# Giuseppe5/brevitas

Measured on AMD Instinct MI355X. Metric: Gelem/s fused int8 fake-quant fwd+bwd, per-channel, [256,512,56,56], higher is better.
Workload: dtype bf16

## Files before the change

brevitas_amd/_native.py:

```python
import ctypes
import os

import torch

_PKG = os.path.dirname(os.path.abspath(__file__))
LIB_PATH = os.environ.get('BREVITAS_AMD_LIB') or os.path.join(_PKG, 'libbvq.so')

F32, BF16, F16 = 0, 1, 2
ROUND, FLOOR, CEIL, ROUND_TO_ZERO, DPU_ROUND = range(5)
(OP_ROUND, OP_FLOOR, OP_CEIL, OP_ROUND_TO_ZERO, OP_DPU_ROUND, OP_BINARY_SIGN, OP_TERNARY_SIGN,
 OP_ABS) = range(8)
STAT_ABSMAX, STAT_MINMAX = 0, 1
SCALAR_OPMATH, SCALAR_CAST = 0, 1
OUT_DEQUANT, OUT_INT = 0, 1
MATCH_ABS, MATCH_VALUE = 0, 1
MATCH_FIRST = 16
PRE_NONE, PRE_RELU, PRE_SIGMOID, PRE_TANH = 0, 1, 2, 3
CODES_I32, CODES_I8, CODES_U8 = 0, 1, 2
CLUSTER_FORCE_FALLBACK = 1
_CODES_TORCH = {CODES_I32: torch.int32, CODES_I8: torch.int8, CODES_U8: torch.uint8}
ABI_VERSION = 2

_DTYPES = {torch.float32: F32, torch.bfloat16: BF16, torch.float16: F16}

EXPORTS = (
    'bvq_abi_version', 'bvq_last_error', 'bvq_unary', 'bvq_stats_pre', 'bvq_scalar_clamp', 'bvq_tensor_clamp',
    'bvq_tensor_clamp_bwd', 'bvq_abs_binary_sign_grad_bwd', 'bvq_stats_workspace_bytes', 'bvq_stats',
    'bvq_absmax_scale', 'bvq_running_stats_update', 'bvq_scale_from_stat', 'bvq_shard_pack', 'bvq_shard_unpack', 'bvq_abs_moments_workspace_bytes', 'bvq_abs_moments',
    'bvq_abs_affine_bwd', 'bvq_kth_workspace_bytes', 'bvq_kth_value', 'bvq_kth_pair', 'bvq_kth_passes',
    'bvq_kth_hist_offset', 'bvq_kth_begin', 'bvq_kth_hist', 'bvq_kth_pick', 'bvq_kth_finish', 'bvq_stat_bwd', 'bvq_tie_info_bytes', 'bvq_stat_tie_scan', 'bvq_stat_tie_apply', 'bvq_stat_tie_apply_dscale', 'bvq_fakequant_fwd', 'bvq_stats_fakequant_fwd_workspace_bytes', 'bvq_stats_fakequant_fwd',
    'bvq_fakequant_bwd_workspace_bytes', 'bvq_fakequant_bwd_stats_workspace_bytes', 'bvq_fakequant_bwd_stats', 'bvq_fakequant_bwd',
    'bvq_learned_scale', 'bvq_fakequant_bwd_learned', 'bvq_variant_fwd', 'bvq_variant_bwd_workspace_bytes', 'bvq_variant_bwd',
    'bvq_fakequant_fwd_bounds', 'bvq_fakequant_bwd_bounds', 'bvq_histc', 'bvq_absmax_scale_running', 'bvq_selftest_div_f16r',
    'bvq_kthw_plan', 'bvq_kthw_begin', 'bvq_kthw_hist', 'bvq_kthw_pick', 'bvq_kthw_finish',
    'bvq_absmax_onepass_supported', 'bvq_absmax_scale_onepass', 'bvq_fakequant_bwd_stats_onepass_supported',
    'bvq_fakequant_bwd_stats_onepass', 'bvq_scale_from_stat_running', 'bvq_fakequant_bwd_shard',
    'bvq_shard_unpack_deposit', 'bvq_absmax_list_supported', 'bvq_absmax_scale_list', 'bvq_weight_list_supported',
    'bvq_weight_quant_list_fwd', 'bvq_weight_quant_list_bwd_workspace_bytes', 'bvq_weight_quant_list_bwd',
    'bvq_absmax_fakequant_cluster_supported', 'bvq_absmax_fakequant_cluster', 'bvq_selftest_pre_op')


class QuantDesc(ctypes.Structure):
    _fields_ = [
        ('outer', ctypes.c_int64), ('channels', ctypes.c_int64), ('inner', ctypes.c_int64),
        ('x_dtype', ctypes.c_int32), ('ct_dtype', ctypes.c_int32), ('scale_dtype', ctypes.c_int32),
        ('zp_dtype', ctypes.c_int32), ('scale_per_channel', ctypes.c_int32),
        ('zp_per_channel', ctypes.c_int32), ('qmin', ctypes.c_float), ('qmax', ctypes.c_float),
        ('round_mode', ctypes.c_int32), ('scalar_mode', ctypes.c_int32), ('clamp_ste', ctypes.c_int32),
        ('out_kind', ctypes.c_int32), ('pre_op', ctypes.c_int32), ('codes_dtype', ctypes.c_int32)]


class VariantDesc(ctypes.Structure):
    _fields_ = [
        ('outer', ctypes.c_int64), ('channels', ctypes.c_int64), ('inner', ctypes.c_int64), ('kind', ctypes.c_int32),
        ('x_dtype', ctypes.c_int32), ('ct_dtype', ctypes.c_int32), ('scale_dtype', ctypes.c_int32),
        ('zp_dtype', ctypes.c_int32), ('scale_per_channel', ctypes.c_int32), ('round_mode', ctypes.c_int32),
        ('clamp_ste', ctypes.c_int32), ('scalar_mode', ctypes.c_int32), ('qmin', ctypes.c_float),
        ('qmax', ctypes.c_float), ('threshold', ctypes.c_float), ('trunc_scale', ctypes.c_float)]


VAR_BINARY, VAR_CLAMPED_BINARY, VAR_TERNARY, VAR_DECOUPLED, VAR_TRUNC = range(5)

WEIGHT_LIST_MAX = 16


class WeightItem(ctypes.Structure):
    _fields_ = [
        ('x', ctypes.c_void_p), ('y', ctypes.c_void_p), ('stat', ctypes.c_void_p), ('scale', ctypes.c_void_p),
        ('g', ctypes.c_void_p), ('dx', ctypes.c_void_p), ('dscale', ctypes.c_void_p), ('channels', ctypes.c_int64),
        ('inner', ctypes.c_int64), ('min_val', ctypes.c_double), ('int_threshold', ctypes.c_double),
        ('qmin', ctypes.c_float), ('qmax', ctypes.c_float), ('use_min', ctypes.c_int32), ('clamp_ste', ctypes.c_int32)]

# ... 51 lines not shown
        'bvq_kth_pair': (i32, [i32, i32, vp, i64, i64, i64, i64, i64, vp, vp, i64, vp]),
        'bvq_kth_passes': (i32, [i32]),
        'bvq_kth_hist_offset': (i64, [i32, i64, i32]),
        'bvq_kth_begin': (i32, [i32, i64, i32, i64, dbl, vp, i64, vp]),
        'bvq_kth_hist': (i32, [i32, i32, vp, i64, i64, i64, i32, vp, i64, vp]),
        'bvq_kth_pick': (i32, [i32, i64, i32, i32, dbl, vp, i64, vp]),
        'bvq_kth_finish': (i32, [i32, i32, i64, vp, vp, i64, vp]),
        'bvq_kthw_plan': (i32, [i32, i32, i32, vp, vp]),
        'bvq_kthw_begin': (i32, [i32, i32, vp, i64, vp]),
        'bvq_kthw_hist': (i32, [i32, i32, vp, i64, i32, vp, i64, vp]),
        'bvq_kthw_pick': (i32, [i32, i32, i32, i32, i64, dbl, vp, i64, vp]),
        'bvq_kthw_finish': (i32, [i32, i32, vp, vp, i64, vp]),
        'bvq_tie_info_bytes': (i64, [i64]),
        'bvq_stat_tie_scan': (i32, [i32, i32, vp, vp, i64, i64, i64, vp, vp, vp]),
        'bvq_stat_tie_apply': (i32, [i32, i32, i32, vp, vp, vp, vp, vp, vp, i64, i64, i64, i32, vp]),
        'bvq_stat_tie_apply_dscale': (i32, [i32, i32, vp, vp, vp, i32, dbl, i32, vp, vp, vp, i64, i64, i64, vp]),
        'bvq_fakequant_bwd': (i32, [ctypes.POINTER(QuantDesc), vp, vp, vp, vp, vp, vp, vp, vp, vp, vp, i64, vp]),
        'bvq_learned_scale': (i32, [i32, vp, i64, dbl, i32, dbl, i32, vp, vp]),
        'bvq_histc': (i32, [i32, vp, i64, vp, i32, vp, vp]),
        'bvq_selftest_div_f16r': (i32, [vp, i32, vp, i32, vp, vp]),
        'bvq_selftest_pre_op': (i32, [i32, i32, vp, vp, vp, vp, i64, vp]),
        'bvq_fakequant_fwd_bounds': (i32, [ctypes.POINTER(QuantDesc), vp, vp, vp, vp, vp, vp]),
        'bvq_fakequant_bwd_bounds': (i32, [ctypes.POINTER(QuantDesc), vp, vp, vp, vp, vp, vp, vp, vp, vp, i64, vp]),
        'bvq_variant_fwd': (i32, [ctypes.POINTER(VariantDesc), vp, vp, vp, vp, vp, vp, vp]),
        'bvq_variant_bwd_workspace_bytes': (i64, [ctypes.POINTER(VariantDesc)]),
        'bvq_variant_bwd': (i32, [ctypes.POINTER(VariantDesc), vp, vp, vp, vp, vp, vp, vp, vp, vp, vp, i64, vp]),
        'bvq_weight_list_supported': (i32, [i32, i32, i32, vp, i64]),
        'bvq_weight_quant_list_fwd': (i32, [i32, i32, i32, i32, vp, vp]),
        'bvq_weight_quant_list_bwd_workspace_bytes': (i64, [i32, i32, vp]),
        'bvq_weight_quant_list_bwd': (i32, [i32, i32, i32, i32, i32, vp, vp, i64, vp, i64, vp]),
        'bvq_absmax_fakequant_cluster_supported': (i64, [ctypes.POINTER(QuantDesc), vp, vp]),
        'bvq_absmax_fakequant_cluster': (i32, [ctypes.POINTER(QuantDesc), vp, dbl, i32, dbl, vp, vp, i32, vp, dbl, i32, vp,
                                               vp, i64, i32, vp, vp]),
        'bvq_fakequant_bwd_learned': (i32, [ctypes.POINTER(QuantDesc), vp, vp, vp, vp, vp, vp, vp, i32, dbl, i32, dbl, vp, vp, vp, i64, vp]),
    }
    for name, (res, args) in sig.items():
        fn = getattr(lib, name, None)
        if fn is None:
            if strict:
                raise ImportError('brevitas_amd: %s does not export %s' % (path, name))
            continue
        fn.restype = res
        fn.argtypes = args
    ver = lib.bvq_abi_version()
    if ver != ABI_VERSION:
        raise ImportError('brevitas_amd: libbvq.so has ABI %d, this package needs %d' % (ver, ABI_VERSION))
    return lib


lib = _load()


def last_error():
    return lib.bvq_last_error().decode()


def check(rc, what):
    if rc != 0:
        raise BvqError('%s failed (%d): %s' % (what, rc, last_error()))


def dtype_code(dtype):
    try:
        return _DTYPES[dtype]
    except KeyError:
        raise BvqError('brevitas_amd: unsupported dtype %s (float32, bfloat16, float16)' % dtype)
# ... 197 lines not shown
            _timer.before('bvq_fakequant_fwd')
        check(lib.bvq_fakequant_fwd(ctypes.byref(desc), ptr(x), ptr(scale), ptr(zp), ptr(y), ptr(codes),
                                    stream_ptr(dev)), 'bvq_fakequant_fwd')
        if _timer is not None:
            _timer.after('bvq_fakequant_fwd')
    if not want_y:
        return codes
    return (y, codes) if want_codes else y


def stats_fakequant_fwd(desc, x, min_val, int_threshold, scale_dtype):
    dev = require_device(x)
    assert x.is_contiguous()
    y = torch.empty_like(x)
    wsb = int(lib.bvq_stats_fakequant_fwd_workspace_bytes(ctypes.byref(desc), ptr(x), ptr(y)))
    if wsb <= 0:
        return None
    channels = int(desc.channels) if (desc.scale_per_channel and desc.channels > 1) else 1
    stat = torch.empty(channels, dtype=x.dtype, device=dev)
    scale = torch.empty(channels, dtype=scale_dtype, device=dev)
    ws = torch.empty(wsb, dtype=torch.uint8, device=dev)
    with _DeviceGuard(dev):
        if _timer is not None:
            _timer.before('bvq_stats_fakequant_fwd')
        check(lib.bvq_stats_fakequant_fwd(ctypes.byref(desc), ptr(x), float(min_val or 0.0), int(bool(min_val)),
                                          float(int_threshold), ptr(stat), ptr(scale), ptr(y), ptr(ws), wsb,
                                          stream_ptr(dev)), 'bvq_stats_fakequant_fwd')
        if _timer is not None:
            _timer.after('bvq_stats_fakequant_fwd')
    return stat, scale, y


def absmax_fakequant_cluster(desc, x, min_val, int_threshold, scale_dtype, running=None, momentum=0.0,
                             first_batch=False, flags=0, fallbacks=None):
    dev = require_device(x)
    assert x.is_contiguous()
    y = torch.empty_like(x)
    words = int(lib.bvq_absmax_fakequant_cluster_supported(ctypes.byref(desc), ptr(x), ptr(y)))
    if words <= 0:
        return None
    with _DeviceGuard(dev):
        st = stream_ptr(dev)
        arrive = arrival_buffer(dev, st, words)
        if arrive is None:
            return None
        stat = torch.empty(desc.channels, dtype=x.dtype, device=dev)
        scale = torch.empty(desc.channels, dtype=scale_dtype, device=dev)
        if _timer is not None:
            _timer.before('bvq_stats_fakequant_fwd')
        check(lib.bvq_absmax_fakequant_cluster(
            ctypes.byref(desc), ptr(x), float(min_val or 0.0), int(bool(min_val)), float(int_threshold), ptr(stat),
            ptr(scale), dtype_code(running.dtype) if running is not None else 0, ptr(running), float(momentum),
            int(first_batch), ptr(y), ptr(arrive), arrive.numel(), int(flags), ptr(fallbacks), st),
            'bvq_absmax_fakequant_cluster')
        if _timer is not None:
            _timer.after('bvq_stats_fakequant_fwd')
    return stat, scale, y


def absmax_scale_list(xs, outers, channels, inners, min_val, int_threshold, scale_dtype):
    dev = require_device(*xs)
    n = len(xs)
    dt = dtype_code(xs[0].dtype)
    for x, o, i in zip(xs, outers, inners):
        assert x.is_contiguous() and x.dtype == xs[0].dtype and x.numel() == o * channels * i
    ptrs = (ctypes.c_void_p * n)(*[x.data_ptr() for x in xs])
    oa = (ctypes.c_int64 * n)(*outers)
    ia = (ctypes.c_int64 * n)(*inners)
    if not lib.bvq_absmax_list_supported(dt, n, ptrs, oa, channels, ia):
        return None
    with _DeviceGuard(dev):
        st = stream_ptr(dev)
        arrive = ws = None
        if channels > 1:
            arrive = arrival_buffer(dev, st, max(2 * channels, 18))
            if arrive is None:
                return None
        else:
            ws = torch.empty(1 << 14, dtype=torch.uint8, device=dev)
        stat = torch.empty(channels, dtype=xs[0].dtype, device=dev)
        scale = torch.empty(channels, dtype=scale_dtype, device=dev)
        check(lib.bvq_absmax_scale_list(dt, n, ptrs, oa, channels, ia, ptr(stat), float(min_val or 0.0),
                                        int(bool(min_val)), float(int_threshold), dtype_code(scale_dtype), ptr(scale),
                                        ptr(arrive), arrive.numel() if arrive is not None else 0, ptr(ws),
                                        ws.numel() if ws is not None else 0, st), 'bvq_absmax_scale_list')
    return stat, scale

# ... 578 lines not shown
```

brevitas_amd/csrc/bvq_fakequant_fwd.hip:

```cpp

#include "bvq_act.h"
#include "bvq_fakequant.h"
#include "bvq_stat_epilogue.h"

namespace bvq {

template <typename CT, int RM, bool ZP0, typename Div>
__device__ __forceinline__ float fwd_elem(float xf, const Div& div, float s, float z, float qmin,
                                          float qmax, bool out_int, int mode, float& q_out) {
  float t = rnd<CT>(div(xf));
  t = ZP0 ? t + 0.f : rnd<CT>(t + z);
  t = do_round<CT, RM>(t, mode);
  const float q = clamp_where(t, qmin, qmax);
  q_out = q;
  if (out_int) return q;
  return ZP0 ? rnd<CT>(q * s) : rnd<CT>(rnd<CT>(q - z) * s);
}

template <typename CT, int RM, bool ZP0, typename Div, typename S>
__device__ __forceinline__ f2 fwd_elem2(f2 xf, const Div& div, S s, S z, float qmin, float qmax,
                                        bool out_int, int mode, f2& q_out) {
  f2 t = rnd2<CT>(div(xf));
  t = ZP0 ? t + 0.f : rnd2<CT>(t + z);
  t = do_round2<CT, RM>(t, mode);
// ... 243 lines not shown
  int32_t use_min, scale_dtype, scale_pc, scalar_cast, round_mode, pre_relu;
};

template <typename T>
__device__ __forceinline__ float scale_from_key(uint32_t key, bool use_min, float min_val, float int_threshold,
                                                int scale_dtype, float& stat) {
  if constexpr (elem<T>::id == BVQ_F16)
    stat = (float)__builtin_bit_cast(f16_t, (uint16_t)key);
  else
    stat = __builtin_bit_cast(float, key);
  const float thr = (use_min && stat < min_val) ? min_val : stat;
  float s = thr / int_threshold;
  if (scale_dtype == BVQ_BF16)
    s = rnd<bf16_t>(s);
  else if (scale_dtype == BVQ_F16)
    s = rnd<f16_t>(s);
  return s;
}
template <typename T>
__device__ __forceinline__ void store_stat_scale(void* stat_out, void* scale_out, int scale_dtype, int32_t c,
                                                 float stat, float s) {
  if constexpr (elem<T>::id == BVQ_F32)
    reinterpret_cast<float*>(stat_out)[c] = stat;
  else
    reinterpret_cast<T*>(stat_out)[c] = (T)stat;
  if (scale_dtype == BVQ_F32)
    reinterpret_cast<float*>(scale_out)[c] = s;
  else if (scale_dtype == BVQ_BF16)
    reinterpret_cast<bf16_t*>(scale_out)[c] = (bf16_t)s;
  else
    reinterpret_cast<f16_t*>(scale_out)[c] = (f16_t)s;
}

template <typename T, int RM, bool PRE, typename Div>
__device__ __forceinline__ void fused_quantize(const vec_t<T, elem<T>::vec> (&xv)[kFusedSlots], const bool (&ok)[kFusedSlots],
                                               T* __restrict__ yp, int lane, const Div& div, float s,
                                               float qmin, float qmax, int mode) {
  constexpr int VEC = elem<T>::vec;
  constexpr bool ZP0 = sizeof(T) == 2;
#pragma unroll
  for (int j = 0; j < kFusedSlots; ++j) {
    if (ok[j]) {
      vec_t<T, VEC> yv;
#pragma unroll
      for (int k = 0; k < VEC; k += 2) {
        f2 xf = widen2<T>(xv[j].v[k], xv[j].v[k + 1]);
        if constexpr (PRE) xf = relu2(xf);
        f2 q2;
        const f2 r = fwd_elem2<T, RM, ZP0>(xf, div, s, 0.f, qmin, qmax, false, mode, q2);
        pack2<T>(r, yv.v[k], yv.v[k + 1]);
      }
      store_vec<T, VEC, true>(yp + (int64_t)(lane + kWave * j) * VEC, yv);
    }
  }
}

__global__ void fused_zero_kernel(uint32_t* p, int64_t n) {
  const int64_t i = (int64_t)blockIdx.x * blockDim.x + threadIdx.x;
  if (i < n) p[i] = 0u;
}

__device__ __forceinline__ void fused_slice(const FusedArgs& a, int q, int lane, int& r, int& sl, bool (&ok)[kFusedSlots]) {
  const bool active = q < a.slices;
  r = active ? q / a.spr : 0;
  sl = active ? q - r * a.spr : 0;
  const int nch = active ? (a.cpr - sl * kFusedSliceChunks < kFusedSliceChunks ? a.cpr - sl * kFusedSliceChunks
                                                                              : kFusedSliceChunks)
                         : 0;
#pragma unroll
  for (int j = 0; j < kFusedSlots; ++j) ok[j] = lane + kWave * j < nch;
}

template <typename T>
__device__ __forceinline__ void fused_load(const FusedArgs& a, int32_t c, int r, int sl, const bool (&ok)[kFusedSlots],
                                           int lane, vec_t<T, elem<T>::vec> (&xv)[kFusedSlots]) {
  constexpr int VEC = elem<T>::vec;
  const int64_t base = ((int64_t)r * a.channels + c) * a.inner + (int64_t)sl * kFusedSliceChunks * VEC;
  const T* __restrict__ xp = reinterpret_cast<const T*>(a.x) + base;
#pragma unroll
  for (int j = 0; j < kFusedSlots; ++j)
    xv[j] = load_vec<T, VEC, true>(ok[j] ? xp + (int64_t)(lane + kWave * j) * VEC : reinterpret_cast<const T*>(a.x));
}

template <typename T>
__device__ __forceinline__ uint32_t fused_key(const FusedArgs& a, const vec_t<T, elem<T>::vec> (&xv)[kFusedSlots],
                                              const bool (&ok)[kFusedSlots]) {
  uint32_t m = 0;
#pragma unroll
  for (int j = 0; j < kFusedSlots; ++j) {
    if (ok[j]) {
#pragma unroll
      for (int k = 0; k < elem<T>::vec; ++k) {
        const uint32_t b = a.pre_relu ? pre_abs_bits<T, true>(xv[j].v[k]) : pre_abs_bits<T, false>(xv[j].v[k]);
        m = b > m ? b : m;
      }
    }
  }
  return m;
}

template <typename T, int RM>
__device__ __forceinline__ void fused_apply(const FusedArgs& a, int32_t c, int r, int sl,
                                            const vec_t<T, elem<T>::vec> (&xv)[kFusedSlots], const bool (&ok)[kFusedSlots],
                                            float s, float qmin, float qmax, int lane) {
  constexpr int VEC = elem<T>::vec;
  const int64_t base = ((int64_t)r * a.channels + c) * a.inner + (int64_t)sl * kFusedSliceChunks * VEC;
  T* __restrict__ yp = reinterpret_cast<T*>(a.y) + base;
  const int mode = a.round_mode;
  if constexpr (elem<T>::id == BVQ_BF16) {
    if (bf16_scale_ok(s)) {
      const DivBf16 div{1.0f / s};
      if (a.pre_relu)
        fused_quantize<T, RM, true>(xv, ok, yp, lane, div, s, qmin, qmax, mode);
      else
        fused_quantize<T, RM, false>(xv, ok, yp, lane, div, s, qmin, qmax, mode);
      return;
    }
  }
  if constexpr (elem<T>::id == BVQ_F16) {
    if (f16_scale_ok(s)) {
      const DivF16R div{s, 1.0f / s};
      if (a.pre_relu)
        fused_quantize<T, RM, true>(xv, ok, yp, lane, div, s, qmin, qmax, mode);
      else
        fused_quantize<T, RM, false>(xv, ok, yp, lane, div, s, qmin, qmax, mode);
      return;
    }
  }
  const DivExact div{s};
  if (a.pre_relu)
    fused_quantize<T, RM, true>(xv, ok, yp, lane, div, s, qmin, qmax, mode);
  else
    fused_quantize<T, RM, false>(xv, ok, yp, lane, div, s, qmin, qmax, mode);
}

template <typename T, int RM>
// ... 33 lines not shown
    fused_channel<T, RM>(a, c, r, sl, ok, qmin, qmax, wave, lane, nwaves, sh_max, sh_stat);
}

struct FusedListArgs {
  FusedArgs a[BVQ_WEIGHT_LIST_MAX];
  int32_t start[BVQ_WEIGHT_LIST_MAX + 1];
  int32_t n;
};
static_assert(sizeof(FusedListArgs) <= 4096, "kernel arguments are limited to 4 KiB");

template <typename T, int RM>
__global__ __launch_bounds__(kFusedMaxWaves * kWave) void fused_list_fakequant_kernel(FusedListArgs la) {
  __shared__ uint32_t sh_max[kFusedMaxWaves];
  __shared__ uint32_t sh_stat;
  const int lane = threadIdx.x & 63;
  const int wave = __builtin_amdgcn_readfirstlane((int)(threadIdx.x >> 6));
  const int nwaves = (int)(blockDim.x >> 6);
  int p = -1, r = 0, sl = 0;
  bool ok[kFusedSlots];
  float qmin = 0.f, qmax = 0.f;
  for (int32_t pair = blockIdx.x; pair < la.start[la.n]; pair += gridDim.x) {
    if (p < 0 || pair >= la.start[p + 1]) {
      if (p < 0) p = 0;
      while (p + 1 < la.n && pair >= la.start[p + 1]) ++p;
      fused_slice(la.a[p], wave, lane, r, sl, ok);
      qmin = rnd<T>(la.a[p].qmin);
      qmax = rnd<T>(la.a[p].qmax);
    }
    fused_channel<T, RM>(la.a[p], pair - la.start[p], r, sl, ok, qmin, qmax, wave, lane, nwaves, sh_max, sh_stat);
  }
}


#ifndef BVQ_CLUSTER_WAVES
#define BVQ_CLUSTER_WAVES 16
#endif
#ifndef BVQ_CLUSTER_WAVES_PER_CU
#define BVQ_CLUSTER_WAVES_PER_CU 16
#endif
#ifndef BVQ_CLUSTER_PREFETCH
#define BVQ_CLUSTER_PREFETCH 1
#endif
constexpr int kClusterWaves = BVQ_CLUSTER_WAVES;
constexpr int kClusterWavesPerCu = BVQ_CLUSTER_WAVES_PER_CU;
constexpr bool kClusterPrefetch = BVQ_CLUSTER_PREFETCH != 0;
constexpr int kClusterMaxMembers = kWave;
constexpr uint32_t kClusterTag = 0x80000000u;
constexpr uint64_t kClusterBudgetTicks = 200000;
static_assert(kClusterWaves >= 1 && kClusterWaves * kWave <= 1024, "BVQ_CLUSTER_WAVES");

struct ClusterArgs {
  FusedArgs f;
  ScaleEpilogue ep;
  void* stat_out;
  int32_t in_dtype;
  uint32_t* key;
  uint32_t* dep;
  uint32_t* fallbacks;
  int32_t members, nclusters, force_fallback;
};

template <typename T, int RM>
__global__ __launch_bounds__(kClusterWaves * kWave, kClusterWavesPerCu / 4) void cluster_absmax_fakequant_kernel(ClusterArgs ca) {
  constexpr int VEC = elem<T>::vec;
  __shared__ uint32_t sh_max[kClusterWaves];
  __shared__ uint32_t sh_stat, sh_ok;
  const FusedArgs& a = ca.f;
  const int lane = threadIdx.x & 63;
  const int wave = __builtin_amdgcn_readfirstlane((int)(threadIdx.x >> 6));
  const int32_t members = ca.members;
  const int32_t member = (int32_t)blockIdx.x % members, cluster = (int32_t)blockIdx.x / members;
  int r, sl;
  bool ok[kFusedSlots];
  fused_slice(a, member * kClusterWaves + wave, lane, r, sl, ok);
  const float qmin = rnd<T>(a.qmin), qmax = rnd<T>(a.qmax);
  int32_t c = cluster;
  if (c >= a.channels) return;
  vec_t<T, VEC> xv[kFusedSlots];
  fused_load<T>(a, c, r, sl, ok, lane, xv);
  for (; c < a.channels; c += ca.nclusters) {
    const uint32_t m = wave_max_u32(fused_key<T>(a, xv, ok));
    if (lane == 0) sh_max[wave] = m;
    __syncthreads();
    uint32_t* const keys = ca.key + (int64_t)c * members;
    if (wave == 0) {
      uint32_t bm = 0;
      for (int w = 0; w < kClusterWaves; ++w) bm = sh_max[w] > bm ? sh_max[w] : bm;
      if (lane == 0) __hip_atomic_store(keys + member, bm | kClusterTag, __ATOMIC_RELAXED, __HIP_MEMORY_SCOPE_AGENT);
    }
    const int32_t cn = c + ca.nclusters;
    vec_t<T, VEC> xn[kFusedSlots];
    if (kClusterPrefetch && cn < a.channels) fused_load<T>(a, cn, r, sl, ok, lane, xn);
    if (wave == 0) {
      bool done = false;
      uint32_t v = 0;
      if (!ca.force_fallback) {
        const uint64_t t0 = __builtin_amdgcn_s_memrealtime();
        for (;;) {
          v = lane < members ? __hip_atomic_load(keys + lane, __ATOMIC_RELAXED, __HIP_MEMORY_SCOPE_AGENT) : kClusterTag;
          if (__all((v & kClusterTag) != 0)) {
            done = true;
            break;
          }
          if (__builtin_amdgcn_s_memrealtime() - t0 > kClusterBudgetTicks) break;
          __builtin_amdgcn_s_sleep(2);
        }
      }
      v = wave_max_u32(v) & ~kClusterTag;
      if (lane == 0) {
        sh_stat = v;
        sh_ok = done ? 1u : 0u;
      }
    }
    __syncthreads();
    if (!sh_ok) {
      uint32_t fm = 0;
      for (int q = wave; q < a.slices; q += kClusterWaves) {
        int fr, fsl;
        bool fok[kFusedSlots];
        fused_slice(a, q, lane, fr, fsl, fok);
        const T* xp = reinterpret_cast<const T*>(a.x) + ((int64_t)fr * a.channels + c) * a.inner +
                      (int64_t)fsl * kFusedSliceChunks * VEC;
        for (int j = 0; j < kFusedSlots; ++j) {
          if (!fok[j]) break;
          const vec_t<T, VEC> u = load_vec<T, VEC, false>(xp + (int64_t)(lane + kWave * j) * VEC);
#pragma unroll
          for (int k = 0; k < VEC; ++k) {
            const uint32_t b = a.pre_relu ? pre_abs_bits<T, true>(u.v[k]) : pre_abs_bits<T, false>(u.v[k]);
            fm = b > fm ? b : fm;
          }
        }
      }
      fm = wave_max_u32(fm);
      if (lane == 0) sh_max[wave] = fm;
      __syncthreads();
      if (threadIdx.x == 0) {
        uint32_t bm = 0;
        for (int w = 0; w < kClusterWaves; ++w) bm = sh_max[w] > bm ? sh_max[w] : bm;
        sh_stat = bm;
        if (ca.fallbacks) __hip_atomic_fetch_add(ca.fallbacks, 1u, __ATOMIC_RELAXED, __HIP_MEMORY_SCOPE_AGENT);
      }
      __syncthreads();
    }
    const uint32_t key = sh_stat;
    uint32_t before = 0;
    if (wave == 0) {
      if (lane == 0) {
        if (!sh_ok) asm volatile("s_waitcnt vmcnt(0)" ::: "memory");
        before = __hip_atomic_fetch_add(ca.dep + c, 1u, __ATOMIC_RELAXED, __HIP_MEMORY_SCOPE_AGENT);
      }
    }
    float stat;
    const float s = scale_from_key<T>(key, a.use_min, a.min_val, a.int_threshold, a.scale_dtype, stat);
    if (member == 0 && threadIdx.x == 0) absmax_epilogue(ca.stat_out, ca.in_dtype, ca.in_dtype, ca.ep, c, key);
    fused_apply<T, RM>(a, c, r, sl, xv, ok, s, qmin, qmax, lane);
    if (wave == 0) {
      before = __builtin_amdgcn_readfirstlane(before);
      if (before + 1 == (uint32_t)members) {
        if (lane < members) __hip_atomic_store(keys + lane, 0u, __ATOMIC_RELAXED, __HIP_MEMORY_SCOPE_AGENT);
        if (lane == 0) __hip_atomic_store(ca.dep + c, 0u, __ATOMIC_RELAXED, __HIP_MEMORY_SCOPE_AGENT);
      }
    }
    if (cn < a.channels) {
      if constexpr (kClusterPrefetch) {
#pragma unroll
        for (int j = 0; j < kFusedSlots; ++j) xv[j] = xn[j];
      } else {
        fused_load<T>(a, cn, r, sl, ok, lane, xv);
      }
    }
  }
}

}

using namespace bvq;

static int fakequant_fwd_impl(const bvq_quant_desc* d, const void* x, const void* scale, const void* zp, void* y,
                             void* codes, const float* bounds, bvq_stream_t stream) {
  int rc = validate(d, true);
  if (rc) return rc;
  const bool act = d->pre_op >= BVQ_PRE_SIGMOID;
  if (act && (codes || bounds || !y || d->out_kind != BVQ_OUT_DEQUANT || d->x_dtype != d->ct_dtype)) {
    set_error("bvq_fakequant_fwd: pre_op %d needs the dequantized output in x's dtype, no codes, no device bounds",
              d->pre_op);
    return BVQ_ERR_UNSUPPORTED;
  }
  const int64_t n = d->outer * d->channels * d->inner;
  if (n == 0) return BVQ_OK;
  if (!x || !scale || !zp || (!y && !codes)) {
    set_error("bvq_fakequant_fwd: null pointer");
    return BVQ_ERR_INVALID;
  }
  if (y && !codes && !bounds && !act) {
    const ColsPlan cp = cols_quant_plan(d, x, y, nullptr, true, false, kColsFwdVec16);
    if (cp.ok) {
      ColsQuantArgs ca = {};
      fill_cols_args(ca, cp, d);
      ca.x = x;
      ca.y = y;
      ca.scale = scale;
      ca.zp = zp;
      hipStream_t cst = (hipStream_t)stream;
      const bool cnt = n * (int64_t)(2 * dtype_size(d->x_dtype)) >= nt_threshold_bytes();
      rc = with_cols_variant(d, cnt, [&](auto t, auto rm, auto ntc) {
// ... 146 lines not shown
  a.pre_relu = d->pre_op == BVQ_PRE_RELU;
  return a;
}

extern "C" int bvq_stats_fakequant_fwd(const bvq_quant_desc* d, const void* x, double min_val, int use_min,
                                       double int_threshold, void* stat_out, void* scale_out, void* y,
                                       void* workspace, int64_t workspace_bytes, bvq_stream_t stream) {
  int rc = validate(d);
  if (rc) return rc;
  if (!x || !y || !stat_out || !scale_out || !workspace) {
    set_error("bvq_stats_fakequant_fwd: null pointer");
    return BVQ_ERR_INVALID;
  }
  hipStream_t st = (hipStream_t)stream;
  FusedPlan p;
  if (fused_plan(d, x, y, p)) {
    const FusedArgs a = fused_args(d, p, x, y, stat_out, scale_out, min_val, use_min, int_threshold);
    const dim3 grid((unsigned)p.nblocks), block((unsigned)(p.waves * kWave));
    rc = with_cols_variant(d, false, [&](auto t, auto rm, auto) {
      fused_absmax_fakequant_kernel<typename decltype(t)::type, rm><<<grid, block, 0, st>>>(a);
    });
    return rc ? rc : check_launch("bvq_stats_fakequant_fwd");
  }
  set_error("bvq_stats_fakequant_fwd: shape / layout not covered by the one-launch form");
  return BVQ_ERR_UNSUPPORTED;
}

struct ClusterPlan {
  FusedPlan p;
  int32_t members, nclusters;
  int64_t words;
};

static bool cluster_plan(const bvq_quant_desc* d, const void* x, const void* y, ClusterPlan& cp) {
  if (!(d->scale_per_channel && d->channels > 1) || d->channels >= ((int64_t)1 << 31)) return false;
  const FusedShape f = fused_shape(d, x, y);
  if (!f.ok) return false;
  const uintptr_t bytes = (uintptr_t)(f.outer * f.channels * f.inner * dtype_size(d->x_dtype));
  const uintptr_t xa = reinterpret_cast<uintptr_t>(x), ya = reinterpret_cast<uintptr_t>(y);
  if (xa < ya + bytes && ya < xa + bytes) return false;
  const int64_t cpr = f.inner / f.vec;
  const int64_t spr = (cpr + kFusedSliceChunks - 1) / kFusedSliceChunks;
  const int64_t slices = f.outer * spr;
  const int64_t members = (slices + kClusterWaves - 1) / kClusterWaves;
  if (cpr > (1 << 30) || members > kClusterMaxMembers) return false;
  cp.p.cpr = (int32_t)cpr;
  cp.p.spr = (int32_t)spr;
  cp.p.slices = (int32_t)slices;
  cp.p.waves = kClusterWaves;
  cp.members = (int32_t)members;
  const int64_t resident = (int64_t)num_cus() * kClusterWavesPerCu / kClusterWaves;
  int64_t nc = resident / members;
  nc = nc < 1 ? 1 : (nc > f.channels ? f.channels : nc);
  cp.nclusters = (int32_t)nc;
  cp.p.nblocks = (int32_t)(nc * members);
  cp.words = f.channels * (members + 1);
  return true;
}

extern "C" int64_t bvq_absmax_fakequant_cluster_supported(const bvq_quant_desc* d, const void* x, const void* y) {
  if (validate(d)) return 0;
  ClusterPlan cp;
  return cluster_plan(d, x, y, cp) ? cp.words : 0;
}

extern "C" int bvq_absmax_fakequant_cluster(const bvq_quant_desc* d, const void* x, double min_val, int use_min,
                                            double int_threshold, void* stat_out, void* scale_out, int run_dtype,
                                            void* running, double momentum, int first_batch, void* y, uint32_t* arrive,
                                            int64_t arrive_words, int flags, uint32_t* fallbacks,
                                            bvq_stream_t stream) {
  int rc = validate(d);
  if (rc) return rc;
  if (!x || !y || !stat_out || !scale_out || !arrive) {
    set_error("bvq_absmax_fakequant_cluster: null pointer");
    return BVQ_ERR_INVALID;
  }
  auto bad_dtype = [](int dt) { return dt < BVQ_F32 || dt > BVQ_F16; };
  if ((running && bad_dtype(run_dtype)) || bad_dtype(d->scale_dtype) || !(int_threshold == int_threshold) ||
      (flags & ~BVQ_CLUSTER_FORCE_FALLBACK)) {
    set_error("bvq_absmax_fakequant_cluster: bad argument");
    return BVQ_ERR_INVALID;
  }
  ClusterPlan cp;
  if (!cluster_plan(d, x, y, cp)) {
    set_error("bvq_absmax_fakequant_cluster: shape / layout not covered (bvq_absmax_fakequant_cluster_supported)");
    return BVQ_ERR_UNSUPPORTED;
  }
  if (arrive_words < cp.words) {
    set_error("bvq_absmax_fakequant_cluster: arrival buffer of %lld words, %lld needed", (long long)arrive_words,
              (long long)cp.words);
    return BVQ_ERR_WORKSPACE;
  }
  ClusterArgs ca = {};
  ca.f = fused_args(d, cp.p, x, y, stat_out, scale_out, min_val, use_min, int_threshold);
  ca.ep.scale_out = scale_out;
  ca.ep.scale_dtype = d->scale_dtype;
  ca.ep.use_min = use_min;
  ca.ep.min_val = ca.f.min_val;
  ca.ep.int_threshold = ca.f.int_threshold;
  if (running) {
    ca.ep.running = running;
    ca.ep.run_dtype = run_dtype;
    ca.ep.first_batch = first_batch;
    ca.ep.one_minus_m = (float)(1.0 - momentum);
    ca.ep.momentum = (float)momentum;
  }
  ca.stat_out = stat_out;
  ca.in_dtype = d->x_dtype;
  ca.key = arrive;
  ca.dep = arrive + (int64_t)ca.f.channels * cp.members;
  ca.fallbacks = fallbacks;
  ca.members = cp.members;
  ca.nclusters = cp.nclusters;
  ca.force_fallback = (flags & BVQ_CLUSTER_FORCE_FALLBACK) ? 1 : 0;
  hipStream_t st = (hipStream_t)stream;
  rc = with_cols_variant(d, false, [&](auto t, auto rm, auto) {
    cluster_absmax_fakequant_kernel<typename decltype(t)::type, rm><<<dim3((unsigned)cp.p.nblocks), dim3(kClusterWaves * kWave), 0, st>>>(ca);
  });
  return rc ? rc : check_launch("bvq_absmax_fakequant_cluster");
}

namespace bvq {
int fused_list_fwd(int n, const bvq_quant_desc* descs, const bvq_weight_item* items, hipStream_t st) {
  FusedListArgs la = {};
  la.n = n;
  int64_t pairs = 0;
  int waves = 1;
  for (int i = 0; i < n; ++i) {
    const bvq_weight_item& it = items[i];
    FusedPlan p;
    if (!fused_plan(&descs[i], it.x, it.y, p)) {
      set_error("bvq_weight_quant_list_fwd: item %d not covered by the one-launch form", i);
      return BVQ_ERR_UNSUPPORTED;
    }
    la.a[i] = fused_args(&descs[i], p, it.x, it.y, it.stat, it.scale, it.min_val, it.use_min, it.int_threshold);
    la.start[i] = (int32_t)pairs;
    pairs += la.a[i].channels;
    waves = p.waves > waves ? p.waves : waves;
  }
  if (pairs >= ((int64_t)1 << 31)) {
    set_error("bvq_weight_quant_list_fwd: too many channels");
    return BVQ_ERR_UNSUPPORTED;
  }
  la.start[n] = (int32_t)pairs;
  const int64_t budget = (int64_t)num_cus() * 2 * kFusedMaxWaves / waves;
  const dim3 grid((unsigned)(budget < pairs ? budget : pairs)), block((unsigned)(waves * kWave));
  const int rc = with_cols_variant(&descs[0], false, [&](auto t, auto rm, auto) {
    fused_list_fakequant_kernel<typename decltype(t)::type, rm><<<grid, block, 0, st>>>(la);
  });
  return rc ? rc : check_launch("bvq_weight_quant_list_fwd");
}
}
// ... 57 lines not shown
```

include/bvq.h:

```cpp
#ifndef BVQ_H_
#define BVQ_H_

#include <stddef.h>
#include <stdint.h>

#ifdef __cplusplus
extern "C" {
#endif

#define BVQ_ABI_VERSION 2

typedef void* bvq_stream_t;

typedef enum bvq_status {
  BVQ_OK = 0,
  BVQ_ERR_INVALID = -1,
  BVQ_ERR_UNSUPPORTED = -2,
  BVQ_ERR_WORKSPACE = -3,
  BVQ_ERR_LAUNCH = -4
} bvq_status;

typedef enum bvq_dtype { BVQ_F32 = 0, BVQ_BF16 = 1, BVQ_F16 = 2 } bvq_dtype;

typedef enum bvq_round_mode {
// ... 163 lines not shown

int bvq_stat_bwd(int match, int dtype, const void* x, const void* stat, const void* gstat, void* dx,
                 int64_t outer, int64_t channels, int64_t inner, int mode_add, void* workspace,
                 int64_t workspace_bytes, bvq_stream_t stream);

int64_t bvq_tie_info_bytes(int64_t channels);
int bvq_stat_tie_scan(int match, int dtype, const void* x, const void* stat, int64_t outer,
                      int64_t channels, int64_t inner, void* dx_zero_fill, int64_t* tie_info,
                      bvq_stream_t stream);
int bvq_stat_tie_apply(int match, int pre_op, int dtype, const void* x, const void* stat,
                       const void* gstat, const int64_t* tie_info, const int64_t* total_ties, void* dx,
                       int64_t outer, int64_t channels, int64_t inner, int mode_add, bvq_stream_t stream);

int bvq_stat_tie_apply_dscale(int pre_op, int dtype, const void* x, const void* stat, const float* dscale,
                              int scale_dtype, double int_threshold, int quot_dtype,
                              const int64_t* tie_info, const int64_t* total_ties, void* dx, int64_t outer,
                              int64_t channels, int64_t inner, bvq_stream_t stream);


int bvq_fakequant_fwd(const bvq_quant_desc* desc, const void* x, const void* scale, const void* zp,
                      void* y, void* codes, bvq_stream_t stream);

int64_t bvq_stats_fakequant_fwd_workspace_bytes(const bvq_quant_desc* desc, const void* x, const void* y);
int bvq_stats_fakequant_fwd(const bvq_quant_desc* desc, const void* x, double min_val, int use_min,
                            double int_threshold, void* stat_out, void* scale_out, void* y, void* workspace,
                            int64_t workspace_bytes, bvq_stream_t stream);

#define BVQ_CLUSTER_FORCE_FALLBACK 1
int64_t bvq_absmax_fakequant_cluster_supported(const bvq_quant_desc* desc, const void* x, const void* y);
int bvq_absmax_fakequant_cluster(const bvq_quant_desc* desc, const void* x, double min_val, int use_min,
                                 double int_threshold, void* stat_out, void* scale_out, int run_dtype, void* running,
                                 double momentum, int first_batch, void* y, uint32_t* arrive, int64_t arrive_words,
                                 int flags, uint32_t* fallbacks, bvq_stream_t stream);

int64_t bvq_fakequant_bwd_workspace_bytes(const bvq_quant_desc* desc);

int bvq_fakequant_bwd(const bvq_quant_desc* desc, const void* g, const void* x, const void* scale,
                      const void* zp, void* dx, float* dscale, float* dzp, const void* tie_stat,
                      int64_t* tie_info, void* workspace, int64_t workspace_bytes, bvq_stream_t stream);

int bvq_fakequant_fwd_bounds(const bvq_quant_desc* desc, const void* x, const void* scale, const void* zp,
                             const float* bounds, void* y, bvq_stream_t stream);
int bvq_fakequant_bwd_bounds(const bvq_quant_desc* desc, const void* g, const void* x, const void* scale,
                             const void* zp, const float* bounds, void* dx, float* dscale, float* dbounds,
                             void* workspace, int64_t workspace_bytes, bvq_stream_t stream);

int bvq_learned_scale(int value_dtype, const void* value, int64_t n, double min_val, int use_min,
                      double int_threshold, int scale_dtype, void* scale_out, bvq_stream_t stream);
int bvq_fakequant_bwd_learned(const bvq_quant_desc* desc, const void* g, const void* x, const void* scale,
                              const void* zp, void* dx, float* dscale, const void* value, int value_dtype,
                              double min_val, int use_min, double int_threshold, const void* gscale,
                              void* dvalue, void* workspace, int64_t workspace_bytes, bvq_stream_t stream);

int64_t bvq_fakequant_bwd_stats_workspace_bytes(const bvq_quant_desc* desc);
int bvq_fakequant_bwd_stats(const bvq_quant_desc* desc, const void* g, const void* x, const void* scale,
                            const void* zp, const void* stat, void* dx, float* dscale, int scale_dtype,
                            double int_threshold, int quot_dtype, void* workspace, int64_t workspace_bytes,
                            bvq_stream_t stream);

int bvq_fakequant_bwd_stats_onepass_supported(const bvq_quant_desc* d);
int bvq_fakequant_bwd_stats_onepass(const bvq_quant_desc* d, const void* g, const void* x, const void* scale,
                                    const void* zp, const void* stat, void* dx, float* dscale, int scale_dtype,
                                    double int_threshold, int quot_dtype, void* workspace, int64_t workspace_bytes,
                                    uint32_t* arrive, int64_t arrive_words, bvq_stream_t stream);

typedef enum bvq_variant_kind {
// ... 58 lines not shown
```

Baseline: 548.6.

## Add one-shot cluster form, DPP wave max, and count-based slots to cluster absmax fakequant

Reworks the cluster absmax+fakequant kernel. A plan-time choice picks a one-shot form (one cluster per channel, many more blocks) over the walking form when there are many channels and rows are wide. It also replaces the wave max reduction with DPP plus readlane, swaps the per-slot bool array for a count-based predicate, and drops the register-heavy next-channel prefetch. It adds a BF16 round-mode switch and optional timestamp instrumentation, and lowers the launch-bounds occupancy hint. The one-shot form trades the persistent walk for a larger grid, and removing the prefetch may expose load latency in walk mode.

```diff
diff --git a/brevitas_amd/_native.py b/brevitas_amd/_native.py
--- a/brevitas_amd/_native.py
+++ b/brevitas_amd/_native.py
@@ -18,6 +18,7 @@
 PRE_NONE, PRE_RELU, PRE_SIGMOID, PRE_TANH = 0, 1, 2, 3
 CODES_I32, CODES_I8, CODES_U8 = 0, 1, 2
 CLUSTER_FORCE_FALLBACK = 1
+CLUSTER_AUTO, CLUSTER_WALK, CLUSTER_ONESHOT = range(3)
 _CODES_TORCH = {CODES_I32: torch.int32, CODES_I8: torch.int8, CODES_U8: torch.uint8}
 ABI_VERSION = 2
 
@@ -37,7 +38,8 @@
     'bvq_fakequant_bwd_stats_onepass', 'bvq_scale_from_stat_running', 'bvq_fakequant_bwd_shard',
     'bvq_shard_unpack_deposit', 'bvq_absmax_list_supported', 'bvq_absmax_scale_list', 'bvq_weight_list_supported',
     'bvq_weight_quant_list_fwd', 'bvq_weight_quant_list_bwd_workspace_bytes', 'bvq_weight_quant_list_bwd',
-    'bvq_absmax_fakequant_cluster_supported', 'bvq_absmax_fakequant_cluster', 'bvq_selftest_pre_op')
+    'bvq_absmax_fakequant_cluster_supported', 'bvq_absmax_fakequant_cluster', 'bvq_absmax_fakequant_cluster_form',
+    'bvq_selftest_pre_op')
 
 
 class QuantDesc(ctypes.Structure):
@@ -155,6 +157,8 @@
         'bvq_absmax_fakequant_cluster_supported': (i64, [ctypes.POINTER(QuantDesc), vp, vp]),
         'bvq_absmax_fakequant_cluster': (i32, [ctypes.POINTER(QuantDesc), vp, dbl, i32, dbl, vp, vp, i32, vp, dbl, i32, vp,
                                                vp, i64, i32, vp, vp]),
+        'bvq_absmax_fakequant_cluster_form': (i32, [ctypes.POINTER(QuantDesc), vp, dbl, i32, dbl, vp, vp, i32, vp, dbl, i32,
+                                                    vp, vp, i64, i32, vp, i32, vp, vp]),
         'bvq_fakequant_bwd_learned': (i32, [ctypes.POINTER(QuantDesc), vp, vp, vp, vp, vp, vp, vp, i32, dbl, i32, dbl, vp, vp, vp, i64, vp]),
     }
     for name, (res, args) in sig.items():
@@ -418,7 +422,7 @@
 
 
 def absmax_fakequant_cluster(desc, x, min_val, int_threshold, scale_dtype, running=None, momentum=0.0,
-                             first_batch=False, flags=0, fallbacks=None):
+                             first_batch=False, flags=0, fallbacks=None, form=CLUSTER_AUTO, stamps=None):
     dev = require_device(x)
     assert x.is_contiguous()
     y = torch.empty_like(x)
@@ -434,11 +438,14 @@
         scale = torch.empty(desc.channels, dtype=scale_dtype, device=dev)
         if _timer is not None:
             _timer.before('bvq_stats_fakequant_fwd')
-        check(lib.bvq_absmax_fakequant_cluster(
-            ctypes.byref(desc), ptr(x), float(min_val or 0.0), int(bool(min_val)), float(int_threshold), ptr(stat),
-            ptr(scale), dtype_code(running.dtype) if running is not None else 0, ptr(running), float(momentum),
-            int(first_batch), ptr(y), ptr(arrive), arrive.numel(), int(flags), ptr(fallbacks), st),
-            'bvq_absmax_fakequant_cluster')
+        args = (ctypes.byref(desc), ptr(x), float(min_val or 0.0), int(bool(min_val)), float(int_threshold), ptr(stat),
+                ptr(scale), dtype_code(running.dtype) if running is not None else 0, ptr(running), float(momentum),
+                int(first_batch), ptr(y), ptr(arrive), arrive.numel(), int(flags), ptr(fallbacks))
+        if form == CLUSTER_AUTO and stamps is None:
+            check(lib.bvq_absmax_fakequant_cluster(*args, st), 'bvq_absmax_fakequant_cluster')
+        else:
+            check(lib.bvq_absmax_fakequant_cluster_form(*args, int(form), ptr(stamps), st),
+                  'bvq_absmax_fakequant_cluster_form')
         if _timer is not None:
             _timer.after('bvq_stats_fakequant_fwd')
     return stat, scale, y
diff --git a/brevitas_amd/csrc/bvq_fakequant_fwd.hip b/brevitas_amd/csrc/bvq_fakequant_fwd.hip
--- a/brevitas_amd/csrc/bvq_fakequant_fwd.hip
+++ b/brevitas_amd/csrc/bvq_fakequant_fwd.hip
@@ -299,8 +299,8 @@
     reinterpret_cast<f16_t*>(scale_out)[c] = (f16_t)s;
 }
 
-template <typename T, int RM, bool PRE, typename Div>
-__device__ __forceinline__ void fused_quantize(const vec_t<T, elem<T>::vec> (&xv)[kFusedSlots], const bool (&ok)[kFusedSlots],
+template <typename T, int RM, bool PRE, typename Div, typename Ok>
+__device__ __forceinline__ void fused_quantize(const vec_t<T, elem<T>::vec> (&xv)[kFusedSlots], const Ok& ok,
                                                T* __restrict__ yp, int lane, const Div& div, float s,
                                                float qmin, float qmax, int mode) {
   constexpr int VEC = elem<T>::vec;
@@ -349,9 +349,33 @@
     xv[j] = load_vec<T, VEC, true>(ok[j] ? xp + (int64_t)(lane + kWave * j) * VEC : reinterpret_cast<const T*>(a.x));
 }
 
+struct SlotCount {
+  int lane, nch;
+  __device__ __forceinline__ bool operator[](int j) const { return lane + kWave * j < nch; }
+};
+__device__ __forceinline__ void fused_slice(const FusedArgs& a, int q, int lane, int& r, int& sl, SlotCount& ok) {
+  const bool active = q < a.slices;
+  r = active ? q / a.spr : 0;
+  sl = active ? q - r * a.spr : 0;
+  const int left = a.cpr - sl * kFusedSliceChunks;
+  ok.lane = lane;
+  ok.nch = active ? (left < kFusedSliceChunks ? left : kFusedSliceChunks) : 0;
+}
 template <typename T>
+__device__ __forceinline__ void fused_load(const FusedArgs& a, int32_t c, int r, int sl, const SlotCount& ok, int lane,
+                                           vec_t<T, elem<T>::vec> (&xv)[kFusedSlots]) {
+  constexpr int VEC = elem<T>::vec;
+  const int64_t base = ((int64_t)r * a.channels + c) * a.inner + (int64_t)sl * kFusedSliceChunks * VEC;
+  const T* __restrict__ xp = reinterpret_cast<const T*>(a.x) + base;
+  asm volatile("" : "+v"(lane));
+#pragma unroll
+  for (int j = 0; j < kFusedSlots; ++j)
+    xv[j] = load_vec<T, VEC, true>(xp + (lane + kWave * j < ok.nch ? (uint32_t)(lane + kWave * j) * VEC : 0u));
+}
+
+template <typename T, typename Ok>
 __device__ __forceinline__ uint32_t fused_key(const FusedArgs& a, const vec_t<T, elem<T>::vec> (&xv)[kFusedSlots],
-                                              const bool (&ok)[kFusedSlots]) {
+                                              const Ok& ok) {
   uint32_t m = 0;
 #pragma unroll
   for (int j = 0; j < kFusedSlots; ++j) {
@@ -365,10 +389,27 @@
   }
   return m;
 }
-
-template <typename T, int RM>
+template <typename T, std::enable_if_t<sizeof(T) == 4, int> = 0>
+__device__ __forceinline__ uint32_t fused_key(const FusedArgs& a, const vec_t<T, elem<T>::vec> (&xv)[kFusedSlots],
+                                              const SlotCount& ok) {
+  uint32_t m = 0;
+#pragma unroll
+  for (int j = 0; j < kFusedSlots; ++j) {
+    uint32_t mj = 0;
+#pragma unroll
+    for (int k = 0; k < elem<T>::vec; ++k) {
+      const uint32_t b = a.pre_relu ? pre_abs_bits<T, true>(xv[j].v[k]) : pre_abs_bits<T, false>(xv[j].v[k]);
+      mj = b > mj ? b : mj;
+    }
+    mj = ok[j] ? mj : 0u;
+    m = mj > m ? mj : m;
+  }
+  return m;
+}
+
+template <typename T, int RM, typename Ok>
 __device__ __forceinline__ void fused_apply(const FusedArgs& a, int32_t c, int r, int sl,
-                                            const vec_t<T, elem<T>::vec> (&xv)[kFusedSlots], const bool (&ok)[kFusedSlots],
+                                            const vec_t<T, elem<T>::vec> (&xv)[kFusedSlots], const Ok& ok,
                                             float s, float qmin, float qmax, int lane) {
   constexpr int VEC = elem<T>::vec;
   const int64_t base = ((int64_t)r * a.channels + c) * a.inner + (int64_t)sl * kFusedSliceChunks * VEC;
@@ -468,22 +509,11 @@
 }
 
 
-#ifndef BVQ_CLUSTER_WAVES
-#define BVQ_CLUSTER_WAVES 16
-#endif
-#ifndef BVQ_CLUSTER_WAVES_PER_CU
-#define BVQ_CLUSTER_WAVES_PER_CU 16
-#endif
-#ifndef BVQ_CLUSTER_PREFETCH
-#define BVQ_CLUSTER_PREFETCH 1
-#endif
-constexpr int kClusterWaves = BVQ_CLUSTER_WAVES;
-constexpr int kClusterWavesPerCu = BVQ_CLUSTER_WAVES_PER_CU;
-constexpr bool kClusterPrefetch = BVQ_CLUSTER_PREFETCH != 0;
+constexpr int kClusterWaves = 16;
 constexpr int kClusterMaxMembers = kWave;
 constexpr uint32_t kClusterTag = 0x80000000u;
 constexpr uint64_t kClusterBudgetTicks = 200000;
-static_assert(kClusterWaves >= 1 && kClusterWaves * kWave <= 1024, "BVQ_CLUSTER_WAVES");
+enum { kClusterAuto = 0, kClusterWalk = 1, kClusterOneShot = 2 };
 
 struct ClusterArgs {
   FusedArgs f;
@@ -494,10 +524,65 @@
   uint32_t* dep;
   uint32_t* fallbacks;
   int32_t members, nclusters, force_fallback;
+#ifdef BVQ_CLUSTER_STAMPS
+  uint64_t* stamps;
+#endif
 };
 
+constexpr int kClusterStamps = 6;
+#ifdef BVQ_CLUSTER_STAMPS
+#define BVQ_CLUSTER_STAMP(k) \
+  do {                       \
+    if (wave == 0) tk[k] = __builtin_amdgcn_s_memrealtime(); \
+  } while (0)
+#else
+#define BVQ_CLUSTER_STAMP(k) \
+  do {                       \
+  } while (0)
+#endif
+
+__device__ __forceinline__ uint32_t cluster_wave_max(uint32_t v) {
+#define BVQ_DPP_MAX(ctrl)                                                                       \
+  do {                                                                                          \
+    const uint32_t o = (uint32_t)__builtin_amdgcn_update_dpp(0, (int)v, ctrl, 0xf, 0xf, false); \
+    v = o > v ? o : v;                                                                          \
+  } while (0)
+  BVQ_DPP_MAX(0xB1);
+  BVQ_DPP_MAX(0x4E);
+  BVQ_DPP_MAX(0x141);
+  BVQ_DPP_MAX(0x140);
+#undef BVQ_DPP_MAX
+  const uint32_t a = (uint32_t)__builtin_amdgcn_readlane((int)v, 0), b = (uint32_t)__builtin_amdgcn_readlane((int)v, 16);
+  const uint32_t c = (uint32_t)__builtin_amdgcn_readlane((int)v, 32), d = (uint32_t)__builtin_amdgcn_readlane((int)v, 48);
+  const uint32_t ab = a > b ? a : b, cd = c > d ? c : d;
+  return ab > cd ? ab : cd;
+}
+
+template <typename T>
+__device__ __forceinline__ uint32_t cluster_fallback_key(const FusedArgs& a, int32_t c, int wave, int lane) {
+  constexpr int VEC = elem<T>::vec;
+  uint32_t fm = 0;
+  for (int q = wave; q < a.slices; q += kClusterWaves) {
+    const int fr = q / a.spr, fsl = q - fr * a.spr;
+    const int left = a.cpr - fsl * kFusedSliceChunks;
+    const int nch = left < kFusedSliceChunks ? left : kFusedSliceChunks;
+    const T* xp = reinterpret_cast<const T*>(a.x) + ((int64_t)fr * a.channels + c) * a.inner +
+                  (int64_t)fsl * kFusedSliceChunks * VEC;
+#pragma clang loop unroll(disable)
+    for (int i = lane; i < nch; i += kWave) {
+      const vec_t<T, VEC> u = load_vec<T, VEC, false>(xp + (int64_t)i * VEC);
+#pragma unroll
+      for (int k = 0; k < VEC; ++k) {
+        const uint32_t b = a.pre_relu ? pre_abs_bits<T, true>(u.v[k]) : pre_abs_bits<T, false>(u.v[k]);
+        fm = b > fm ? b : fm;
+      }
+    }
+  }
+  return cluster_wave_max(fm);
+}
+
 template <typename T, int RM>
-__global__ __launch_bounds__(kClusterWaves * kWave, kClusterWavesPerCu / 4) void cluster_absmax_fakequant_kernel(ClusterArgs ca) {
+__global__ __launch_bounds__(kClusterWaves * kWave, 8) void cluster_absmax_fakequant_kernel(ClusterArgs ca) {
   constexpr int VEC = elem<T>::vec;
   __shared__ uint32_t sh_max[kClusterWaves];
   __shared__ uint32_t sh_stat, sh_ok;
@@ -507,16 +592,21 @@
   const int32_t members = ca.members;
   const int32_t member = (int32_t)blockIdx.x % members, cluster = (int32_t)blockIdx.x / members;
   int r, sl;
-  bool ok[kFusedSlots];
+  SlotCount ok;
   fused_slice(a, member * kClusterWaves + wave, lane, r, sl, ok);
   const float qmin = rnd<T>(a.qmin), qmax = rnd<T>(a.qmax);
   int32_t c = cluster;
   if (c >= a.channels) return;
+#ifdef BVQ_CLUSTER_STAMPS
+  uint64_t tk[kClusterStamps] = {};
+#endif
+  BVQ_CLUSTER_STAMP(0);
   vec_t<T, VEC> xv[kFusedSlots];
   fused_load<T>(a, c, r, sl, ok, lane, xv);
   for (; c < a.channels; c += ca.nclusters) {
-    const uint32_t m = wave_max_u32(fused_key<T>(a, xv, ok));
+    const uint32_t m = cluster_wave_max(fused_key<T>(a, xv, ok));
     if (lane == 0) sh_max[wave] = m;
+    BVQ_CLUSTER_STAMP(1);
     __syncthreads();
     uint32_t* const keys = ca.key + (int64_t)c * members;
     if (wave == 0) {
@@ -524,9 +614,8 @@
       for (int w = 0; w < kClusterWaves; ++w) bm = sh_max[w] > bm ? sh_max[w] : bm;
       if (lane == 0) __hip_atomic_store(keys + member, bm | kClusterTag, __ATOMIC_RELAXED, __HIP_MEMORY_SCOPE_AGENT);
     }
+    BVQ_CLUSTER_STAMP(2);
     const int32_t cn = c + ca.nclusters;
-    vec_t<T, VEC> xn[kFusedSlots];
-    if (kClusterPrefetch && cn < a.channels) fused_load<T>(a, cn, r, sl, ok, lane, xn);
     if (wave == 0) {
       bool done = false;
       uint32_t v = 0;
@@ -542,7 +631,7 @@
           __builtin_amdgcn_s_sleep(2);
         }
       }
-      v = wave_max_u32(v) & ~kClusterTag;
+      v = cluster_wave_max(v) & ~kClusterTag;
       if (lane == 0) {
         sh_stat = v;
         sh_ok = done ? 1u : 0u;
@@ -550,24 +639,7 @@
     }
     __syncthreads();
     if (!sh_ok) {
-      uint32_t fm = 0;
-      for (int q = wave; q < a.slices; q += kClusterWaves) {
-        int fr, fsl;
-        bool fok[kFusedSlots];
-        fused_slice(a, q, lane, fr, fsl, fok);
-        const T* xp = reinterpret_cast<const T*>(a.x) + ((int64_t)fr * a.channels + c) * a.inner +
-                      (int64_t)fsl * kFusedSliceChunks * VEC;
-        for (int j = 0; j < kFusedSlots; ++j) {
-          if (!fok[j]) break;
-          const vec_t<T, VEC> u = load_vec<T, VEC, false>(xp + (int64_t)(lane + kWave * j) * VEC);
-#pragma unroll
-          for (int k = 0; k < VEC; ++k) {
-            const uint32_t b = a.pre_relu ? pre_abs_bits<T, true>(u.v[k]) : pre_abs_bits<T, false>(u.v[k]);
-            fm = b > fm ? b : fm;
-          }
-        }
-      }
-      fm = wave_max_u32(fm);
+      const uint32_t fm = cluster_fallback_key<T>(a, c, wave, lane);
       if (lane == 0) sh_max[wave] = fm;
       __syncthreads();
       if (threadIdx.x == 0) {
@@ -578,6 +650,7 @@
       }
       __syncthreads();
     }
+    BVQ_CLUSTER_STAMP(3);
     const uint32_t key = sh_stat;
     uint32_t before = 0;
     if (wave == 0) {
@@ -589,7 +662,24 @@
     float stat;
     const float s = scale_from_key<T>(key, a.use_min, a.min_val, a.int_threshold, a.scale_dtype, stat);
     if (member == 0 && threadIdx.x == 0) absmax_epilogue(ca.stat_out, ca.in_dtype, ca.in_dtype, ca.ep, c, key);
-    fused_apply<T, RM>(a, c, r, sl, xv, ok, s, qmin, qmax, lane);
+    if constexpr (RM == kAnyRM && elem<T>::id == BVQ_BF16) {
+      switch (a.round_mode) {
+#define BVQ_CLUSTER_APPLY(M)                                              \
+  case M:                                                                 \
+    fused_apply<T, M>(a, c, r, sl, xv, ok, s, qmin, qmax, lane); \
+    break
+        BVQ_CLUSTER_APPLY(BVQ_ROUND);
+        BVQ_CLUSTER_APPLY(BVQ_FLOOR);
+        BVQ_CLUSTER_APPLY(BVQ_CEIL);
+        BVQ_CLUSTER_APPLY(BVQ_ROUND_TO_ZERO);
+        default:
+          fused_apply<T, BVQ_DPU_ROUND>(a, c, r, sl, xv, ok, s, qmin, qmax, lane);
+#undef BVQ_CLUSTER_APPLY
+      }
+    } else {
+      fused_apply<T, RM>(a, c, r, sl, xv, ok, s, qmin, qmax, lane);
+    }
+    BVQ_CLUSTER_STAMP(4);
     if (wave == 0) {
       before = __builtin_amdgcn_readfirstlane(before);
       if (before + 1 == (uint32_t)members) {
@@ -597,16 +687,20 @@
         if (lane == 0) __hip_atomic_store(ca.dep + c, 0u, __ATOMIC_RELAXED, __HIP_MEMORY_SCOPE_AGENT);
       }
     }
-    if (cn < a.channels) {
-      if constexpr (kClusterPrefetch) {
-#pragma unroll
-        for (int j = 0; j < kFusedSlots; ++j) xv[j] = xn[j];
-      } else {
-        fused_load<T>(a, cn, r, sl, ok, lane, xv);
-      }
-    }
-  }
-}
+#ifdef BVQ_CLUSTER_STAMPS
+    BVQ_CLUSTER_STAMP(5);
+    if (ca.stamps && wave == 0 && lane < kClusterStamps) {
+      uint64_t t = tk[0];
+#pragma unroll
+      for (int k = 1; k < kClusterStamps; ++k) t = lane == k ? tk[k] : t;
+      ca.stamps[((int64_t)c * members + member) * kClusterStamps + lane] = t;
+    }
+    if (wave == 0) tk[0] = tk[5];
+#endif
+    if (cn < a.channels) fused_load<T>(a, cn, r, sl, ok, lane, xv);
+  }
+}
+#undef BVQ_CLUSTER_STAMP
 
 }
 
@@ -819,7 +913,7 @@
   int64_t words;
 };
 
-static bool cluster_plan(const bvq_quant_desc* d, const void* x, const void* y, ClusterPlan& cp) {
+static bool cluster_plan(const bvq_quant_desc* d, const void* x, const void* y, ClusterPlan& cp, int form = kClusterAuto) {
   if (!(d->scale_per_channel && d->channels > 1) || d->channels >= ((int64_t)1 << 31)) return false;
   const FusedShape f = fused_shape(d, x, y);
   if (!f.ok) return false;
@@ -836,9 +930,15 @@
   cp.p.slices = (int32_t)slices;
   cp.p.waves = kClusterWaves;
   cp.members = (int32_t)members;
-  const int64_t resident = (int64_t)num_cus() * kClusterWavesPerCu / kClusterWaves;
-  int64_t nc = resident / members;
+  int64_t nc = (int64_t)num_cus() * 2 / members;
   nc = nc < 1 ? 1 : (nc > f.channels ? f.channels : nc);
+  if (form == kClusterAuto) {
+    const int64_t row_chunks = cpr < kFusedSliceChunks ? cpr : kFusedSliceChunks;
+    const bool oneshot = f.channels > 4 * nc && 2 * row_chunks >= kFusedSliceChunks;
+    form = oneshot ? kClusterOneShot : kClusterWalk;
+  }
+  if (form == kClusterOneShot && f.channels * members > ((int64_t)1 << 30)) form = kClusterWalk;
+  if (form == kClusterOneShot) nc = f.channels;
   cp.nclusters = (int32_t)nc;
   cp.p.nblocks = (int32_t)(nc * members);
   cp.words = f.channels * (members + 1);
@@ -851,11 +951,10 @@
   return cluster_plan(d, x, y, cp) ? cp.words : 0;
 }
 
-extern "C" int bvq_absmax_fakequant_cluster(const bvq_quant_desc* d, const void* x, double min_val, int use_min,
-                                            double int_threshold, void* stat_out, void* scale_out, int run_dtype,
-                                            void* running, double momentum, int first_batch, void* y, uint32_t* arrive,
-                                            int64_t arrive_words, int flags, uint32_t* fallbacks,
-                                            bvq_stream_t stream) {
+static int cluster_impl(const bvq_quant_desc* d, const void* x, double min_val, int use_min, double int_threshold,
+                        void* stat_out, void* scale_out, int run_dtype, void* running, double momentum, int first_batch,
+                        void* y, uint32_t* arrive, int64_t arrive_words, int flags, uint32_t* fallbacks, int form,
+                        uint64_t* stamps, bvq_stream_t stream) {
   int rc = validate(d);
   if (rc) return rc;
   if (!x || !y || !stat_out || !scale_out || !arrive) {
@@ -868,8 +967,18 @@
     set_error("bvq_absmax_fakequant_cluster: bad argument");
     return BVQ_ERR_INVALID;
   }
+  if (form < kClusterAuto || form > kClusterOneShot) {
+    set_error("bvq_absmax_fakequant_cluster: form %d", form);
+    return BVQ_ERR_INVALID;
+  }
+#ifndef BVQ_CLUSTER_STAMPS
+  if (stamps) {
+    set_error("bvq_absmax_fakequant_cluster: this library was built without BVQ_CLUSTER_STAMPS");
+    return BVQ_ERR_UNSUPPORTED;
+  }
+#endif
   ClusterPlan cp;
-  if (!cluster_plan(d, x, y, cp)) {
+  if (!cluster_plan(d, x, y, cp, form)) {
     set_error("bvq_absmax_fakequant_cluster: shape / layout not covered (bvq_absmax_fakequant_cluster_supported)");
     return BVQ_ERR_UNSUPPORTED;
   }
@@ -900,11 +1009,33 @@
   ca.members = cp.members;
   ca.nclusters = cp.nclusters;
   ca.force_fallback = (flags & BVQ_CLUSTER_FORCE_FALLBACK) ? 1 : 0;
+#ifdef BVQ_CLUSTER_STAMPS
+  ca.stamps = stamps;
+#endif
   hipStream_t st = (hipStream_t)stream;
+  const dim3 grid((unsigned)cp.p.nblocks), block(kClusterWaves * kWave);
   rc = with_cols_variant(d, false, [&](auto t, auto rm, auto) {
-    cluster_absmax_fakequant_kernel<typename decltype(t)::type, rm><<<dim3((unsigned)cp.p.nblocks), dim3(kClusterWaves * kWave), 0, st>>>(ca);
+    cluster_absmax_fakequant_kernel<typename decltype(t)::type, rm><<<grid, block, 0, st>>>(ca);
   });
   return rc ? rc : check_launch("bvq_absmax_fakequant_cluster");
+}
+
+extern "C" int bvq_absmax_fakequant_cluster(const bvq_quant_desc* d, const void* x, double min_val, int use_min,
+                                            double int_threshold, void* stat_out, void* scale_out, int run_dtype,
+                                            void* running, double momentum, int first_batch, void* y, uint32_t* arrive,
+                                            int64_t arrive_words, int flags, uint32_t* fallbacks,
+                                            bvq_stream_t stream) {
+  return cluster_impl(d, x, min_val, use_min, int_threshold, stat_out, scale_out, run_dtype, running, momentum,
+                      first_batch, y, arrive, arrive_words, flags, fallbacks, kClusterAuto, nullptr, stream);
+}
+
+extern "C" int bvq_absmax_fakequant_cluster_form(const bvq_quant_desc* d, const void* x, double min_val, int use_min,
+                                                 double int_threshold, void* stat_out, void* scale_out, int run_dtype,
+                                                 void* running, double momentum, int first_batch, void* y,
+                                                 uint32_t* arrive, int64_t arrive_words, int flags, uint32_t* fallbacks,
+                                                 int form, uint64_t* stamps, bvq_stream_t stream) {
+  return cluster_impl(d, x, min_val, use_min, int_threshold, stat_out, scale_out, run_dtype, running, momentum,
+                      first_batch, y, arrive, arrive_words, flags, fallbacks, form, stamps, stream);
 }
 
 namespace bvq {
diff --git a/include/bvq.h b/include/bvq.h
--- a/include/bvq.h
+++ b/include/bvq.h
@@ -219,6 +219,11 @@
                                  double int_threshold, void* stat_out, void* scale_out, int run_dtype, void* running,
                                  double momentum, int first_batch, void* y, uint32_t* arrive, int64_t arrive_words,
                                  int flags, uint32_t* fallbacks, bvq_stream_t stream);
+int bvq_absmax_fakequant_cluster_form(const bvq_quant_desc* desc, const void* x, double min_val, int use_min,
+                                      double int_threshold, void* stat_out, void* scale_out, int run_dtype,
+                                      void* running, double momentum, int first_batch, void* y, uint32_t* arrive,
+                                      int64_t arrive_words, int flags, uint32_t* fallbacks, int form, uint64_t* stamps,
+                                      bvq_stream_t stream);
 
 int64_t bvq_fakequant_bwd_workspace_bytes(const bvq_quant_desc* desc);
 
```

Measured after the change: 563.6, median of 6. +2.7%, better.
